# twogc/quic-test

Hardware: AMD Instinct MI355X
Metric: FEC encode+decode GiB/s (device-resident), k=10 r=3 1200B pkts, 1/2/4/8 GPU (higher is better)
Workload: dtype u8; 1 GPU; C2 encode + C3 decode: k=10 r=3, 1200 B packets, 1M groups/GPU, 2 erasures/group; k=10, r=3, packet_bytes=1200, groups_per_gpu=1000000, erasures_per_group=2, decode_api=fec_recover_batch_rs_dev (rebuilt packets at (g*r + m)*P slots), parallelism=group-sharded x1 (no collective)

## Files before the change

### quic-test_amd/csrc/fec_kernels.hip

```cpp
#include <hip/hip_runtime.h>

#include <cstdint>
#include <cstdlib>
#include <type_traits>

#include "bitslice.hpp"
#include "coef_tables.hpp"
#include "fec_kernels.hpp"
#include "fec_knobs.hpp"

namespace qfec {
namespace {

struct Tab {
  uint32_t t0lo, t0hi, t1lo, t1hi, t2, coef, p0, p1;
};

typedef uint32_t u32x4 __attribute__((ext_vector_type(4)));
typedef uint32_t u32x4u __attribute__((ext_vector_type(4), aligned(1)));
typedef uint32_t u32u __attribute__((aligned(1)));


template <int POL>
__device__ __forceinline__ u32x4 ld16(const uint8_t* p) {
// ... 462 lines not shown
      for (uint32_t b = 0; b < kBatch; ++b)
        if (s0 + b < k) consume(v[b], s0 + b, k);
    }
  }
#pragma unroll
  for (int m = 0; m < MAXE; ++m) {
    if (m0 + m < e) {
      const uint32_t eid = (POL & kCompactOut) != 0 ? m0 + m : rec_byte(rw, 64 + m0 + m);
      stw<NW, POL>(og + eid * static_cast<uint64_t>(P) + off, acc[m]);
    }
  }
}

template <int K, int MAXE, int POL, int NM, int NT, bool DIRECT, bool INLINE>
__device__ __forceinline__ void fused_group(uint64_t gw, uint64_t m, uint32_t lane, const uint8_t* __restrict__ data,
                                            const uint8_t* __restrict__ parity,
                                            const uint32_t* __restrict__ rec_off,
                                            const uint8_t* __restrict__ codebook, uint32_t P, uint32_t r,
                                            uint32_t m0, uint8_t* __restrict__ out, const RankMeta& rm,
                                            uint8_t* __restrict__ status) {
  constexpr int NW = 4 * NM + NT;
  constexpr uint64_t kmask = (1ull << K) - 1;
  uint64_t rec_byte_off;
  if constexpr (INLINE) {
    uint64_t dm = m & kmask;
    const uint64_t rmask = (1ull << r) - 1;
    const uint64_t pm = (m >> K) & rmask;
    const uint32_t ne = static_cast<uint32_t>(__popcll(dm));
    const bool bad = ne > r - static_cast<uint32_t>(__popcll(pm));
    if (status != nullptr && lane == 0) status[gw] = bad ? 1 : 0;
    if (ne == 0 || bad) return;
    uint64_t rank_e = 0, rank_r = 0;
    for (uint32_t t = 0; dm; ++t) {
      rank_e += choose_small(static_cast<uint32_t>(__builtin_ctzll(dm)), t + 1u);
      dm &= dm - 1;
    }
    uint64_t sp = ~pm & rmask;
    for (uint32_t t = 0; t < ne; ++t) {
      rank_r += choose_small(static_cast<uint32_t>(__builtin_ctzll(sp)), t + 1u);
      sp &= sp - 1;
    }
    rec_byte_off = rm.base[ne] + (rank_e * rm.count_r[ne] + rank_r) * rm.stride[ne];
  } else {
    const uint32_t rec = __builtin_amdgcn_readfirstlane(rec_off[gw]);
    if (rec >= kRecBad) return;
    rec_byte_off = static_cast<uint64_t>(rec) * 32u;
  }
  const uint8_t* recp = codebook + rec_byte_off;
  const uint32_t* rw = reinterpret_cast<const uint32_t*>(recp);
  uint32_t e;
  bool xor_only;
  uint64_t surv = 0, lost = 0;
  if constexpr (DIRECT) {
    lost = m & kmask;
    e = static_cast<uint32_t>(__popcll(lost));
    uint64_t alive = ~(m >> K) & ((r >= 64 ? 0ull : (1ull << r)) - 1);
    xor_only = e == 1 && (alive & 1u);
    uint64_t rsel = 0;
    for (uint32_t t = 0; t < e; ++t) {
      rsel |= alive & (~alive + 1);
      alive &= alive - 1;
    }
    surv = (~lost & kmask) | (rsel << K);
  } else {
    e = rw[24] & 0xFFu;
    xor_only = ((rw[24] >> 8) & 0xFFu) != 0;
  }
  if (m0 >= e) return;
  const Tab* tabs = reinterpret_cast<const Tab*>(recp + 128);
  const uint8_t* dg = data + gw * K * static_cast<uint64_t>(P);
  const uint8_t* pg = parity + gw * r * static_cast<uint64_t>(P);
  uint8_t* og = out + gw * K * static_cast<uint64_t>(P);
  const uint32_t main_end = NM * 1024u;
  uint32_t toff[NT > 0 ? NT : 1];
#pragma unroll
  for (int t = 0; t < NT; ++t) {
    toff[t] = main_end + t * 256u + lane * 4u;
    if (toff[t] + 4u > P) toff[t] = P - 4u;
  }
  auto load = [&](const uint8_t* base, uint32_t (&v)[NW]) {
#pragma unroll
    for (int i = 0; i < NM; ++i) {
      const u32x4 t = ld16<POL>(base + i * 1024u + lane * 16u);
      v[4 * i] = t.x;
      v[4 * i + 1] = t.y;
      v[4 * i + 2] = t.z;
      v[4 * i + 3] = t.w;
    }
#pragma unroll
    for (int t = 0; t < NT; ++t) {
      if constexpr ((POL & kNtLoad) != 0) v[4 * NM + t] = __builtin_nontemporal_load(reinterpret_cast<const u32u*>(base + toff[t]));
      else v[4 * NM + t] = *reinterpret_cast<const u32u*>(base + toff[t]);
    }
  };
  auto store = [&](uint8_t* base, const uint32_t (&v)[NW]) {
#pragma unroll
    for (int i = 0; i < NM; ++i) st16<POL>(base + i * 1024u + lane * 16u, u32x4{v[4 * i], v[4 * i + 1], v[4 * i + 2], v[4 * i + 3]});
#pragma unroll
    for (int t = 0; t < NT; ++t) {
      if constexpr ((POL & kNtStore) != 0) __builtin_nontemporal_store(v[4 * NM + t], reinterpret_cast<u32u*>(base + toff[t]));
      else *reinterpret_cast<u32u*>(base + toff[t]) = v[4 * NM + t];
    }
  };
  auto shard = [&](uint32_t sid) {
    return sid < K ? dg + sid * static_cast<uint64_t>(P) : pg + (sid - K) * static_cast<uint64_t>(P);
  };
  uint32_t sid[K];
#pragma unroll
  for (int s = 0; s < K; ++s) {
    if constexpr (DIRECT) {
      sid[s] = static_cast<uint32_t>(__builtin_ctzll(surv));
      surv &= surv - 1;
    } else {
      sid[s] = rec_byte(rw, s);
    }
  }
  auto dest = [&](uint32_t m, uint32_t eid) -> uint8_t* {
    if constexpr ((POL & kCompactOut) != 0) {
      uint64_t row = gw * r + m;
      if constexpr (INLINE) {
        if (rec_off != nullptr) row = static_cast<uint64_t>(__builtin_amdgcn_readfirstlane(rec_off[gw])) + m;
      }
      return out + row * static_cast<uint64_t>(P);
    } else {
      return og + eid * static_cast<uint64_t>(P);
    }
  };
  auto erased = [&](uint32_t m) -> uint32_t {
    if constexpr (DIRECT) {
      uint64_t x = lost;
      for (uint32_t t = 0; t < m; ++t) x &= x - 1;
      return static_cast<uint32_t>(__builtin_ctzll(x));
    } else {
      return rec_byte(rw, 64 + m);
    }
  };
  if (xor_only) {
    uint32_t acc[NW] = {};
#pragma unroll
    for (int s = 0; s < K; ++s) {
      uint32_t v[NW];
      load(shard(sid[s]), v);
#pragma unroll
      for (int q = 0; q < NW; ++q) acc[q] ^= v[q];
    }
    store(dest(0, erased(0)), acc);
    return;
  }
  constexpr bool kLds = (POL & kLdsTabs) != 0;
  constexpr int kTabPieces = MAXE * K * 2;
  constexpr int kTabIter = kLds ? (kTabPieces + 63) / 64 : 1;
  const uint32_t tab_pieces = (e - m0 < MAXE ? e - m0 : MAXE) * K * 2u;
  constexpr int kSliceTabs = kTabIter * 64 / 2;
  constexpr int kCoefIter = (MAXE * K + 63) / 64;
  uint32_t coef[kCoefIter];
  if constexpr (kLds && (POL & kCoefBytes) != 0) {
    const uint8_t* cb = recp + 128 + m0 * K;
    const uint32_t ncoef = tab_pieces / 2u;
#pragma unroll
    for (int j = 0; j < kCoefIter; ++j) {
      const uint32_t i = lane + 64u * j;
      coef[j] = i < ncoef ? cb[i] : 0u;
    }
  } else if constexpr (kLds) {
    const uint8_t* src = reinterpret_cast<const uint8_t*>(tabs + m0 * K);
    uint8_t* dst = reinterpret_cast<uint8_t*>(wave_tabs_lds<kSliceTabs>());
#pragma unroll
    for (int i = 0; i < kTabIter; ++i) {
      uint32_t idx = lane + 64u * i;
      if (idx >= tab_pieces) idx = tab_pieces - 1u;
      __builtin_amdgcn_global_load_lds(reinterpret_cast<const void*>(src + idx * 16u),
                                       (__attribute__((address_space(3))) void*)(dst + i * 1024), 16, 0, 0);
    }
  }
  constexpr bool kWinPath = kLds;
  constexpr int kWinW = 6;
  constexpr int kWin = kWinPath ? (K < kWinW ? K : kWinW) : K;
  uint32_t x[K][NW];
#pragma unroll
  for (int s = 0; s < kWin; ++s) load(shard(sid[s]), x[s]);
  if constexpr (kLds && (POL & kCoefBytes) != 0) {
    Tab* lt = wave_tabs_lds<kSliceTabs>();
    const uint32_t ncoef = tab_pieces / 2u;
#pragma unroll
    for (int j = 0; j < kCoefIter; ++j) {
      const uint32_t i = lane + 64u * j;
      if (i < ncoef) {
        const TabWords w = tab_words(coef[j]);
        lt[i] = Tab{w.t0lo, w.t0hi, w.t1lo, w.t1hi, w.t2, coef[j], 0u, 0u};
      }
    }
  }
  const Tab* rt = tabs + m0 * K;
  if constexpr (kWinPath) {
    const Tab* lt = rt;
    if constexpr (kLds) {
      __builtin_amdgcn_s_waitcnt(0x0F70);
      __builtin_amdgcn_fence(__ATOMIC_ACQUIRE, "wavefront");
      __builtin_amdgcn_wave_barrier();
      lt = wave_tabs_lds<kSliceTabs>();
    }
    auto rebuild = [&](auto nr_c) __attribute__((always_inline)) {
      constexpr int NR = decltype(nr_c)::value;
      uint32_t acc[NR][NW];
#pragma unroll
      for (int m = 0; m < NR; ++m)
#pragma unroll
        for (int q = 0; q < NW; ++q) acc[m][q] = 0;
#pragma unroll
      for (int s = 0; s < K; ++s) {
#pragma unroll
        for (int q = 0; q < NW; ++q) __asm__ volatile("" : "+v"(x[s][q]));
        __builtin_amdgcn_sched_barrier(0);
        if (s + kWin < K) load(shard(sid[s + kWin]), x[s + kWin]);
        uint32_t s0[NW], s1[NW], s2[NW];
#pragma unroll
        for (int q = 0; q < NW; ++q) {
          s0[q] = x[s][q] & 0x07070707u;
          s1[q] = (x[s][q] >> 3) & 0x07070707u;
          s2[q] = (x[s][q] >> 6) & 0x03030303u;
        }
#pragma unroll
        for (int m = 0; m < NR; ++m) {
          const Tab t = lt[m * K + s];
#pragma unroll
          for (int q = 0; q < NW; ++q) {
            acc[m][q] ^= gmul(s0[q], s1[q], s2[q], t);
            __asm__ volatile("" : "+v"(acc[m][q]));
          }
        }
      }
#pragma unroll
      for (int m = 0; m < NR; ++m) store(dest(m0 + m, erased(m0 + m)), acc[m]);
    };
    for_row_count<MAXE>(e - m0 < MAXE ? e - m0 : MAXE, rebuild);
    return;
  } else {
#pragma unroll
    for (int s = kWin; s < K; ++s) load(shard(sid[s]), x[s]);
  }
  uint32_t acc[MAXE][NW];
#pragma unroll
  for (int m = 0; m < MAXE; ++m)
#pragma unroll
    for (int q = 0; q < NW; ++q) acc[m][q] = 0;
#pragma unroll
  for (int s = 0; s < K; ++s) {
    uint32_t s0[NW], s1[NW], s2[NW];
#pragma unroll
    for (int q = 0; q < NW; ++q) {
      s0[q] = x[s][q] & 0x07070707u;
      s1[q] = (x[s][q] >> 3) & 0x07070707u;
      s2[q] = (x[s][q] >> 6) & 0x03030303u;
    }
#pragma unroll
    for (int m = 0; m < MAXE; ++m) {
      if (m0 + m < e) {
        const Tab& t = rt[m * K + s];
        if (t.coef == 1u) {
#pragma unroll
          for (int q = 0; q < NW; ++q) acc[m][q] ^= x[s][q];
        } else if (t.coef != 0u) {
#pragma unroll
          for (int q = 0; q < NW; ++q) acc[m][q] ^= gmul(s0[q], s1[q], s2[q], t);
        }
      }
    }
  }
#pragma unroll
  for (int m = 0; m < MAXE; ++m)
    if (m0 + m < e) store(dest(m0 + m, erased(m0 + m)), acc[m]);
}

template <int K, int MAXE, int POL, int NM, int NT, bool DIRECT = false, bool INLINE = DIRECT, int SCAN = 0>
__global__ __launch_bounds__(256) void decode_fused(const uint8_t* __restrict__ data,
                                                    const uint8_t* __restrict__ parity,
                                                    const uint32_t* __restrict__ rec_off,
                                                    const uint8_t* __restrict__ codebook,
                                                    uint64_t groups, uint32_t P, uint32_t r, uint32_t m0,
                                                    uint8_t* __restrict__ out, uint32_t never, uint32_t swz,
                                                    const uint64_t* __restrict__ masks, RankMeta rm,
                                                    uint8_t* __restrict__ status) {
  static_assert(!INLINE || (DIRECT && MAXE <= 3), "inline classify: mask-addressed forms with r <= 3");
  static_assert(SCAN == 0 || (DIRECT && INLINE && (SCAN <= 64 || SCAN % 256 == 0)),
                "scan: mask-addressed inline forms, <= 64 groups per wave or whole 256-group rows per block");
  extern __shared__ __attribute__((aligned(16))) uint8_t occupancy_lds[];
  if (never) occupancy_lds[threadIdx.x] = 0;
  const uint64_t wv = static_cast<uint64_t>(decode_block(swz)) * 4u +
                      static_cast<uint32_t>(__builtin_amdgcn_readfirstlane(threadIdx.x >> 6));
  const uint32_t lane = threadIdx.x & 63u;
  if constexpr (SCAN > 64) {
    constexpr int J = SCAN / 256;
    __shared__ uint64_t seg_mask[SCAN];
    __shared__ uint16_t seg_idx[SCAN];
    __shared__ uint32_t seg_cnt[J * 4];
    const uint64_t g0 = static_cast<uint64_t>(decode_block(swz)) * SCAN;
    if (g0 >= groups) return;
    const uint32_t wave = static_cast<uint32_t>(__builtin_amdgcn_readfirstlane(threadIdx.x >> 6));
    constexpr uint64_t kmask = (1ull << K) - 1;
    uint64_t mv[J], bal[J];
#pragma unroll
    for (int j = 0; j < J; ++j) {
      const uint64_t g = g0 + j * 256u + threadIdx.x;
      bool need = false;
      mv[j] = 0;
      if (g < groups) {
        mv[j] = masks[g];
        const uint32_t ne = static_cast<uint32_t>(__popcll(mv[j] & kmask));
        const bool bad = ne > r - static_cast<uint32_t>(__popcll((mv[j] >> K) & ((1ull << r) - 1)));
        if (status != nullptr) status[g] = bad ? 1 : 0;
        need = ne > 0 && !bad;
      }
      bal[j] = __ballot(need);
      if (lane == 0) seg_cnt[j * 4 + wave] = static_cast<uint32_t>(__popcll(bal[j]));
    }
    __syncthreads();
    uint32_t total = 0, off[J];
#pragma unroll
    for (int c = 0; c < J * 4; ++c) {
      if (static_cast<uint32_t>(c % 4) == wave) off[c / 4] = total;
      total += seg_cnt[c];
    }
    const uint64_t below = (1ull << lane) - 1;
#pragma unroll
    for (int j = 0; j < J; ++j) {
      if ((bal[j] >> lane) & 1u) {
        const uint32_t pos = off[j] + static_cast<uint32_t>(__popcll(bal[j] & below));
        seg_mask[pos] = mv[j];
        seg_idx[pos] = static_cast<uint16_t>(j * 256u + threadIdx.x);
      }
    }
    __syncthreads();
    for (uint32_t i = wave; i < total; i += 4u) {
      const uint64_t mi = seg_mask[i];
      const uint64_t m = (static_cast<uint64_t>(__builtin_amdgcn_readfirstlane(static_cast<uint32_t>(mi >> 32))) << 32) |
                         __builtin_amdgcn_readfirstlane(static_cast<uint32_t>(mi));
      const uint32_t gl = __builtin_amdgcn_readfirstlane(static_cast<uint32_t>(seg_idx[i]));
      fused_group<K, MAXE, POL, NM, NT, DIRECT, INLINE>(g0 + gl, m, lane, data, parity, rec_off, codebook, P, r, m0,
                                                        out, rm, nullptr);
    }
  } else if constexpr (SCAN == 0) {
    if (wv >= groups) return;
    const uint64_t m = DIRECT ? masks[wv] : 0;
    fused_group<K, MAXE, POL, NM, NT, DIRECT, INLINE>(wv, m, lane, data, parity, rec_off, codebook, P, r, m0, out, rm,
                                                      status);
  } else {
    const uint64_t g0 = wv * SCAN;
    if (g0 >= groups) return;
    uint64_t mv = 0;
    bool need = false;
    if (lane < static_cast<uint32_t>(SCAN) && g0 + lane < groups) {
      mv = masks[g0 + lane];
      constexpr uint64_t kmask = (1ull << K) - 1;
      const uint32_t ne = static_cast<uint32_t>(__popcll(mv & kmask));
      const bool bad = ne > r - static_cast<uint32_t>(__popcll((mv >> K) & ((1ull << r) - 1)));
      if (status != nullptr) status[g0 + lane] = bad ? 1 : 0;
      need = ne > 0 && !bad;
    }
    uint64_t work = __ballot(need);
    while (work) {
      const uint32_t b = static_cast<uint32_t>(__builtin_ctzll(work));
      work &= work - 1;
      const uint64_t m = (static_cast<uint64_t>(__builtin_amdgcn_readlane(static_cast<uint32_t>(mv >> 32), b)) << 32) |
                         __builtin_amdgcn_readlane(static_cast<uint32_t>(mv), b);
      fused_group<K, MAXE, POL, NM, NT, DIRECT, INLINE>(g0 + b, m, lane, data, parity, rec_off, codebook, P, r, m0,
                                                        out, rm, nullptr);
    }
  }

}

constexpr uint64_t kRunAgg = 1ull << 32;
constexpr uint64_t kRunIncl = 2ull << 32;
constexpr uint32_t kRunEpochShift = 34;

struct RunMeta {
  const Tab* tabs;
// ... 1072 lines not shown
  if (tile == 0) return hipErrorInvalidValue;
  const uint32_t bs = (tile * cpp + 63) / 64 * 64;
  return for_chunks(a.groups, max_wave_blocks() * 2 * tile, [&](uint64_t g0, uint64_t gn) {
    const uint32_t blocks = static_cast<uint32_t>((gn + 2 * tile - 1) / (2 * tile));
    constexpr int kDefWaves = (POL & kStageRows) != 0 ? 10 : 0;
    const int waves = a.waves_per_cu ? a.waves_per_cu : knob(TestKnob::kEncodeWaves, kDefWaves);
    uint32_t smem = occupancy_cap_lds(waves, bs / 64);
    if constexpr ((POL & kStageRows) != 0) smem = std::max<uint32_t>(smem, 2 * tile * R * a.P);
    LaunchRecord t = launch_record(LaunchForm::kEncodeBits, blocks, bs, g0, gn);
    t.k = K, t.r = R, t.off = 0, t.pol = POL, t.tile = tile, t.aux = W;
    trace_launch(t);
    hipLaunchKernelGGL((encode_bits<K, R, W, POL>), dim3(blocks), dim3(bs), smem, s, a.data, a.parity, g0, cpp, a.P,
                       tile, gn, 0u);
  });
}

template <int OFF>
hipError_t run_encode_generic(const EncodeLaunch& a, hipStream_t s) {
  if (a.P < kVecMinP) {
    return for_chunks(a.groups, groups_per_launch(a.P), [&](uint64_t g0, uint64_t gn) {
      const uint32_t n = static_cast<uint32_t>(gn * a.P);
      LaunchRecord t = launch_record(LaunchForm::kEncodeBytes, blocks_for(n), 256, g0, gn);
      t.k = 0, t.off = OFF;
      trace_launch(t);
      hipLaunchKernelGGL(encode_bytes<OFF>, dim3(blocks_for(n)), dim3(256), 0, s, a.data, a.offsets,
                         a.parity, g0, n, a.P, a.k, a.r, static_cast<const Tab*>(a.tables));
    });
  }
  for (uint32_t row0 = 0; row0 < a.r; row0 += 8) {
    const uint32_t rows = (a.r - row0 < 8) ? a.r - row0 : 8;
    hipError_t e = hipSuccess;
#define QFEC_PASS(RR)                                                            \
  case RR:                                                                       \
    e = row0 == 0 ? run_encode_v16<0, RR, OFF, true>(a, row0, s)                 \
                  : run_encode_v16<0, RR, OFF, false>(a, row0, s);               \
    break;
    switch (rows) {
      QFEC_PASS(1)
      QFEC_PASS(2)
      QFEC_PASS(3)
      QFEC_PASS(4)
      QFEC_PASS(5)
      QFEC_PASS(6)
      QFEC_PASS(7)
      QFEC_PASS(8)
      default:
        return hipErrorInvalidValue;
    }
#undef QFEC_PASS
    if (e != hipSuccess) return e;
  }
  return hipSuccess;
}

}

hipError_t launch_encode(const EncodeLaunch& a, hipStream_t s) {
  if (a.groups == 0) return hipSuccess;
  const EncodeForm f = encode_form(a);
  if (f.K == 0)
    return f.OFF == 0 ? run_encode_generic<0>(a, s) : f.OFF == 1 ? run_encode_generic<1>(a, s)
         : f.OFF == 2 ? run_encode_generic<2>(a, s) : run_encode_generic<3>(a, s);
#define QFEC_V16(KK, RR, OO, PP)                                                              \
  if (f.kernel == EncodeKernel::kV16 && f.K == KK && f.R == RR && f.OFF == OO && f.POL == (PP)) \
    return run_encode_v16<KK, RR, OO, true, PP>(a, 0, s);
#define QFEC_BITS(KK, RR, OO, PP)                                                              \
  if (f.kernel == EncodeKernel::kBits && f.K == KK && f.R == RR && f.OFF == OO && f.POL == (PP)) \
    return run_encode_bits<KK, RR, 4, PP>(a, s);
  QFEC_ENCODE_V16_FORMS(QFEC_V16)
  QFEC_ENCODE_BITS_FORMS(QFEC_BITS)
#undef QFEC_BITS
#undef QFEC_V16
  return hipErrorNotSupported;
}

namespace {

RankMeta rank_meta(const LevelMeta& m) {
  RankMeta rm{};
  for (int e = 1; e <= 3; ++e) rm.base[e] = m.base[e], rm.stride[e] = m.stride[e], rm.count_r[e] = m.count_r[e];
  return rm;
}

hipError_t run_classify(const DecodeLaunch& a, hipStream_t s) {
  return for_chunks(a.groups, max_launch_threads(), [&](uint64_t g0, uint64_t gn) {
    trace_launch(launch_record(LaunchForm::kClassify, blocks_for(gn), 256, g0, gn));
    hipLaunchKernelGGL(classify, dim3(blocks_for(gn)), dim3(256), 0, s, a.masks + g0, gn, a.k, a.r,
                       a.binom, a.meta, a.rec_off ? a.rec_off + g0 : nullptr, a.status ? a.status + g0 : nullptr);
  });
}

hipError_t run_decode_bytes(const DecodeLaunch& a, hipStream_t s) {
  return for_chunks(a.groups, groups_per_launch(a.P), [&](uint64_t g0, uint64_t gn) {
    const uint32_t n = static_cast<uint32_t>(gn * a.P);
    LaunchRecord t = launch_record(LaunchForm::kDecodeBytes, blocks_for(n), 256, g0, gn);
    t.k = 0, t.pol = a.compact_out ? kCompactOut : 0;
    trace_launch(t);
    hipLaunchKernelGGL(decode_bytes, dim3(blocks_for(n)), dim3(256), 0, s, a.data, a.parity,
                       a.rec_off, a.codebook, g0, n, a.P, a.k, a.r, a.out ? a.out : a.data,
                       a.compact_out ? 1u : 0u);
  });
}

template <int K, int MAXE>
hipError_t run_decode_v16(const DecodeLaunch& a, hipStream_t s) {
  const uint32_t cpp = (a.P + 15u) / 16u;
  const uint32_t passes = (a.r + MAXE - 1) / MAXE;
  for (uint32_t p = 0; p < passes; ++p) {
    const uint32_t m0 = p * MAXE;
    const hipError_t e = for_chunks(a.groups, max_wave_blocks() * 4, [&](uint64_t g0, uint64_t gn) {
      const uint64_t bn = (gn + 3) / 4;
      LaunchRecord t = launch_record(LaunchForm::kDecodeV16, bn, 256, g0, gn);
      t.k = K, t.r = MAXE, t.aux = m0;
      trace_launch(t);
      hipLaunchKernelGGL((decode_v16<K, MAXE>), dim3(static_cast<uint32_t>(bn)), dim3(256), 0, s,
                         a.data + g0 * a.k * static_cast<uint64_t>(a.P),
                         a.parity + g0 * a.r * static_cast<uint64_t>(a.P), a.rec_off ? a.rec_off + g0 : nullptr, a.codebook,
                         gn, cpp, a.P, a.k, a.r, m0);
    });
    if (e != hipSuccess) return e;
  }
  return hipSuccess;
}

template <int K, int MAXE, int POL>
hipError_t run_decode_wave(const DecodeLaunch& a, hipStream_t s) {
  const uint32_t passes = (a.r + MAXE - 1) / MAXE;
  const uint32_t cap = occupancy_cap_lds(a.waves_per_cu ? a.waves_per_cu : knob(TestKnob::kDecodeWaves, kDecodeWavesPerCU), 4);
  for (uint32_t p = 0; p < passes; ++p) {
    const uint32_t m0 = p * MAXE;
    const uint32_t rows = a.r - m0 < MAXE ? a.r - m0 : MAXE;
    const uint32_t slice = (POL & kLdsTabs) != 0 ? (rows * a.k * 2u + 63u) / 64u * 1024u : 0u;
    const uint32_t smem = cap > 4 * slice ? cap : 4 * slice;
    const hipError_t e = for_chunks(a.groups, max_wave_blocks() * 4, [&](uint64_t g0, uint64_t gn) {
      const uint64_t bn = (gn + 3) / 4;
      LaunchRecord t = launch_record(LaunchForm::kDecodeWave, bn, 256, g0, gn);
      t.k = K, t.r = MAXE, t.pol = POL, t.aux = m0;
      trace_launch(t);
      hipLaunchKernelGGL((decode_wave<K, MAXE, POL>), dim3(static_cast<uint32_t>(bn)), dim3(256), smem, s,
                         a.data + g0 * a.k * static_cast<uint64_t>(a.P),
                         a.parity + g0 * a.r * static_cast<uint64_t>(a.P), a.rec_off ? a.rec_off + g0 : nullptr, a.codebook, gn, a.P,
                         a.k, a.r, m0, (a.out ? a.out : a.data) + g0 * ((POL & kCompactOut) != 0 ? a.r : a.k) * static_cast<uint64_t>(a.P), 0u,
                         decode_swizzle(a, kDecodeWaveXcdSwizzle), slice);
    });
    if (e != hipSuccess) return e;
  }
  return hipSuccess;
}

template <int K, int MAXE, int POL, int NM, int NT, bool DIRECT = false, bool INLINE = DIRECT, int SCAN = 0>
hipError_t run_decode_fused(const DecodeLaunch& a, hipStream_t s) {
  constexpr uint64_t kGroupsPerBlock = SCAN > 64 ? SCAN : 4u * (SCAN > 0 ? SCAN : 1);
  const uint32_t passes = (a.r + MAXE - 1) / MAXE;
  const uint32_t smem = occupancy_cap_lds(a.waves_per_cu ? a.waves_per_cu : knob(TestKnob::kDecodeWaves, kDecodeWavesPerCU), 4);
  const RankMeta rm = rank_meta(a.meta);
  auto out_at = [&](uint64_t g0) -> uint8_t* {
    if (a.packed_rows) return a.out;
    return (a.out ? a.out : a.data) + g0 * ((POL & kCompactOut) != 0 ? a.r : a.k) * static_cast<uint64_t>(a.P);
  };
  for (uint32_t p = 0; p < passes; ++p) {
    const uint32_t m0 = p * MAXE;
    const hipError_t e = for_chunks(a.groups, max_wave_blocks() * kGroupsPerBlock, [&](uint64_t g0, uint64_t gn) {
      const uint64_t bn = (gn + kGroupsPerBlock - 1) / kGroupsPerBlock;
      LaunchRecord t = launch_record(LaunchForm::kDecodeFused, bn, 256, g0, gn);
      t.k = K, t.r = MAXE, t.nm = NM, t.nt = NT, t.pol = POL, t.direct = DIRECT, t.scan = SCAN, t.aux = m0;
      trace_launch(t);
      hipLaunchKernelGGL((decode_fused<K, MAXE, POL, NM, NT, DIRECT, INLINE, SCAN>), dim3(static_cast<uint32_t>(bn)), dim3(256), smem, s,
                         a.data + g0 * a.k * static_cast<uint64_t>(a.P),
                         a.parity + g0 * a.r * static_cast<uint64_t>(a.P), a.rec_off ? a.rec_off + g0 : nullptr, a.codebook, gn, a.P,
                         a.r, m0, out_at(g0), 0u, decode_swizzle(a, kDecodeFusedXcdSwizzle), DIRECT ? a.masks + g0 : nullptr, rm,
                         INLINE && a.status ? a.status + g0 : nullptr);
    });
    if (e != hipSuccess) return e;
  }
  return hipSuccess;
}

template <int K, int MAXE, int POL>
hipError_t run_decode_tiled(const DecodeLaunch& a, uint32_t tile, hipStream_t s) {
  const uint32_t cpp = (a.P + 15u) / 16u;
  const uint32_t bs = (tile * cpp + 63) / 64 * 64;
  return for_chunks(a.groups, groups_per_launch(bs) * tile, [&](uint64_t g0, uint64_t gn) {
    const uint64_t bn = (gn + tile - 1) / tile;
    LaunchRecord t = launch_record(LaunchForm::kDecodeTiled, bn, bs, g0, gn);
    t.k = K, t.r = MAXE, t.pol = POL, t.tile = tile;
    trace_launch(t);
    hipLaunchKernelGGL((decode_tiled<K, MAXE, POL>), dim3(static_cast<uint32_t>(bn)), dim3(bs), 0, s,
                       a.data + g0 * a.k * static_cast<uint64_t>(a.P),
                       a.parity + g0 * a.r * static_cast<uint64_t>(a.P), a.rec_off ? a.rec_off + g0 : nullptr, a.codebook, gn, cpp,
                       a.P, a.r, tile,
                       (a.out ? a.out : a.data) + g0 * ((POL & kCompactOut) != 0 ? a.r : a.k) * static_cast<uint64_t>(a.P));
  });
}

template <DecodeKernel KERNEL, int K, int MAXE, int NM, int NT, int POL, bool DIRECT, int SCAN>
hipError_t run_decode_form(const DecodeLaunch& a, uint32_t tile, hipStream_t s) {
  if constexpr (KERNEL == DecodeKernel::kFused) return run_decode_fused<K, MAXE, POL, NM, NT, DIRECT, DIRECT, SCAN>(a, s);
  else if constexpr (KERNEL == DecodeKernel::kTiled) return run_decode_tiled<K, MAXE, POL>(a, tile, s);
  else if constexpr (KERNEL == DecodeKernel::kWave) return run_decode_wave<K, MAXE, POL>(a, s);
  else if constexpr (KERNEL == DecodeKernel::kV16) return run_decode_v16<K, MAXE>(a, s);
  else return run_decode_bytes(a, s);
}

}

uint64_t rows_prefix_workspace_bytes(uint64_t groups) {
  return ((groups + kRowsPerBlock - 1) / kRowsPerBlock) * sizeof(uint32_t);
}

hipError_t launch_rows_prefix(const uint64_t* masks, uint64_t groups, uint32_t k, uint32_t r, uint32_t* row_start,
                              uint32_t* block_sums, uint64_t* total, hipStream_t s) {
  if (groups == 0) return hipSuccess;
  const uint64_t nb = (groups + kRowsPerBlock - 1) / kRowsPerBlock;
  if (nb > 0xFFFFFFFFull) return hipErrorInvalidValue;
  const uint64_t direct_max = static_cast<uint64_t>(knob(TestKnob::kRowsDirectBlocks, kRowsDirectBlocks));
  const dim3 grid(static_cast<uint32_t>(nb));
  const bool direct = nb <= direct_max;
  {
    trace_launch(launch_record(LaunchForm::kRowsBlockSums, nb, 256, 0, groups));
    if (!direct) trace_launch(launch_record(LaunchForm::kRowsScanBlocks, 1, 256, 0, groups));
    LaunchRecord t = launch_record(LaunchForm::kRowsWrite, nb, 256, 0, groups);
    t.direct = direct;
    trace_launch(t);
  }
  hipLaunchKernelGGL(rows_block_sums, grid, dim3(256), 0, s, masks, groups, k, r, block_sums);
  if (direct) {
    hipLaunchKernelGGL(rows_write<true>, grid, dim3(256), 0, s, masks, groups, k, r, block_sums, row_start, total);
  } else {
    hipLaunchKernelGGL(rows_scan_blocks, dim3(1), dim3(256), 0, s, block_sums, static_cast<uint32_t>(nb), total);
    hipLaunchKernelGGL(rows_write<false>, grid, dim3(256), 0, s, masks, groups, k, r, block_sums, row_start,
                       nullptr);
  }
  return hipGetLastError();
}

namespace {

constexpr int kRunWaves = 8;
constexpr uint32_t kRunGroups = 64u * kRunWaves;

uint64_t runs_blocks_per_launch(uint64_t groups) {
  const uint64_t nb = (groups + kRunGroups - 1) / kRunGroups;
  const uint64_t mb = max_wave_blocks();
  return nb < mb ? nb : mb;
}

template <int K, int R, int NM, int NT, int POL = kNtLoad | kNtStore>
hipError_t run_recover_runs(const RunsLaunch& a, uint32_t stage, hipStream_t s) {
  const RankMeta rm = rank_meta(a.meta);
  uint8_t* ws = static_cast<uint8_t*>(a.workspace);
  uint32_t* ticket = reinterpret_cast<uint32_t*>(ws);
  const uint64_t per = runs_blocks_per_launch(a.groups) * kRunGroups;
  const uint32_t launches = runs_launches(a.groups);
  uint64_t* totals = reinterpret_cast<uint64_t*>(ws + 64);
  uint64_t* lb = reinterpret_cast<uint64_t*>(ws + 64 + 8 * static_cast<uint64_t>(launches));
  return for_chunks(a.groups, per, [&](uint64_t g0, uint64_t gn) {
    const uint32_t c = static_cast<uint32_t>(g0 / per);
    const uint32_t nb = static_cast<uint32_t>((gn + kRunGroups - 1) / kRunGroups);
    LaunchRecord t = launch_record(LaunchForm::kRecoverRuns, nb, 64 * kRunWaves, g0, gn);
    t.k = K, t.r = R, t.nm = NM, t.nt = NT, t.pol = POL, t.tile = kRunGroups, t.aux = stage;
    trace_launch(t);
    hipLaunchKernelGGL((recover_runs<K, R, NM, NT, POL, kRunWaves>), dim3(nb), dim3(64 * kRunWaves), stage, s, a.data + g0 * K * static_cast<uint64_t>(a.P),
                       a.parity + g0 * R * static_cast<uint64_t>(a.P), a.masks + g0, gn, a.P, a.codebook, rm, a.out,
                       a.row_start + g0, a.status ? a.status + g0 : nullptr, lb, ticket, a.epoch + c, stage,
                       c > 0 ? totals + (c - 1) : nullptr, totals + c, c + 1 == launches ? a.total : nullptr, 0u);
  });
}

}

uint32_t runs_launches(uint64_t groups) {
  if (groups == 0) return 0;
  const uint64_t per = runs_blocks_per_launch(groups) * kRunGroups;
  return static_cast<uint32_t>((groups + per - 1) / per);
}

uint64_t runs_workspace_bytes(uint64_t groups) {
  return 64 + 8 * static_cast<uint64_t>(runs_launches(groups)) + 8 * runs_blocks_per_launch(groups);
}

uint32_t runs_stage_bytes(const RunsLaunch& a) {
  if (a.P % 16u != 0 || reinterpret_cast<uintptr_t>(a.out) % 16u != 0) return 0;
  const int v = a.stage_bytes >= 0 ? a.stage_bytes : knob(TestKnob::kRunsStage, kRunsStageBytes);
  if (v <= 0) return 0;
  const uint32_t cap = 64u * 1024u;
  return static_cast<uint32_t>(v) < cap ? static_cast<uint32_t>(v) : cap;
}

hipError_t launch_recover_runs(const RunsLaunch& a, hipStream_t s) {
  if (a.groups == 0) return hipSuccess;
  if (a.workspace == nullptr || a.row_start == nullptr || a.out == nullptr || a.masks == nullptr) return hipErrorInvalidValue;
  if (!runs_supported(a.k, a.r, a.P)) return hipErrorNotSupported;
  const Layout lay = layout_of(a.P);
#define QFEC_RUNS(KK, RR, NMM, NTT) \
  if (a.k == KK && a.r == RR && lay.nm == NMM && lay.nt == NTT) return run_recover_runs<KK, RR, NMM, NTT>(a, runs_stage_bytes(a), s);
  QFEC_RUNS_FORMS(QFEC_RUNS)
#undef QFEC_RUNS
  return hipErrorNotSupported;
}

hipError_t launch_decode(const DecodeLaunch& a, hipStream_t s) {
  const DecodeForm f = decode_form(a);
  if (f.kernel == DecodeKernel::kNone) return hipSuccess;
  if (a.compact_tables != f.compact_tables) return hipErrorInvalidValue;
  if (f.rec_off && a.rec_off == nullptr) return hipErrorInvalidValue;
  if (f.classify) {
    const hipError_t e = run_classify(a, s);
// ... 65 lines not shown
```

### quic-test_amd/csrc/fec_kernels.hpp

```cpp
#pragma once

#include <hip/hip_runtime.h>

#include <cstdint>

#include "fec_forms.hpp"

namespace qfec {

constexpr int kEncodeBlocksPerCU = 2;
constexpr int kEncodeXorWavesPerCU = 15;
constexpr int kDecodeWavesPerCU = 0;

inline uint32_t occupancy_cap_lds(int waves_per_cu, uint32_t waves_per_block) {
  if (waves_per_cu <= 0 || waves_per_block == 0) return 0;
  uint32_t blocks = (static_cast<uint32_t>(waves_per_cu) + waves_per_block / 2) / waves_per_block;
  if (blocks == 0) blocks = 1;
  if (blocks * waves_per_block >= 32) return 0;
  return 160u * 1024u / (blocks + 1) + 16u;
}

constexpr int kDecodeFusedXcdSwizzle = 1;
constexpr int kDecodeWaveXcdSwizzle = 1;

hipError_t launch_encode(const EncodeLaunch& a, hipStream_t s);
hipError_t launch_decode(const DecodeLaunch& a, hipStream_t s);
uint64_t rows_prefix_workspace_bytes(uint64_t groups);
hipError_t launch_rows_prefix(const uint64_t* masks, uint64_t groups, uint32_t k, uint32_t r, uint32_t* row_start,
                              uint32_t* block_sums, uint64_t* total, hipStream_t s);
constexpr int kRunsStageBytes = 48 * 1024;
uint32_t runs_launches(uint64_t groups);
uint64_t runs_workspace_bytes(uint64_t groups);
uint32_t runs_stage_bytes(const RunsLaunch& a);
hipError_t launch_recover_runs(const RunsLaunch& a, hipStream_t s);
constexpr uint32_t kServerSlots = 1024;
constexpr uint32_t kServerMaxGroups = 8;
constexpr uint32_t kServerPackets = 10;
constexpr uint64_t kServerTagShift = 48;
constexpr uint64_t kServerAddrMask = (1ull << kServerTagShift) - 1;
constexpr uint32_t kServerEpoch = 32768;
__host__ __device__ inline uint32_t server_tag(uint64_t seq, uint32_t epoch) {
  return (static_cast<uint32_t>(seq / kServerSlots) & (epoch - 1u)) + 1u;
}
__host__ __device__ inline bool server_scrub_after(uint64_t seq, uint32_t epoch) {
  return (static_cast<uint32_t>(seq / kServerSlots) & (epoch - 1u)) == epoch - 1u;
}
struct alignas(64) ServerSlot {
  uint64_t out;
  uint64_t shape;
  uint64_t addr[kServerMaxGroups * kServerPackets];
};
constexpr uint64_t kServerInline = 1ull << 24;
constexpr uint32_t kInlineMaxGroups = 4;
constexpr uint32_t kInlineMaxP = 1536;
constexpr uint32_t kInlinePayload = 12;
constexpr uint32_t kInlineSlotBytes = kInlineMaxGroups * kServerPackets * (kInlineMaxP / kInlinePayload) * 16;
constexpr uint32_t kServerMaxClasses = 8;
constexpr uint32_t kServerPoll = 16;
struct alignas(64) ServerControl {
  uint64_t stop;
  uint64_t pad0[7];
  uint64_t exited;
  uint64_t pad1[7];
  uint64_t progress[kServerMaxClasses];
  uint64_t bad_slots[kServerMaxClasses];
  uint64_t scrubs[kServerMaxClasses];
};
struct alignas(64) ServerCoord {
  uint64_t leave;
  uint64_t exits;
  uint64_t pad[6];
  uint64_t idle[kServerMaxClasses];
};
__host__ __device__ inline bool server_all_idle(bool idle, const uint64_t* idle_seen, uint32_t classes, uint32_t cls,
                                                uint64_t gen) {
  bool all = idle;
  for (uint32_t c = 0; c < classes; ++c) all = all && (c == cls || idle_seen[c] == gen);
  return all;
}
__host__ __device__ inline uint64_t server_exits_next(uint64_t v, uint64_t gen) {
  return (v >> 8) == gen ? v + 1 : (gen << 8) | 1u;
}
__host__ __device__ inline bool server_exits_last(uint64_t nv, uint32_t classes) { return (nv & 0xFFu) == classes; }
hipError_t launch_legacy_server(ServerSlot* ring, uint8_t* inl, uint64_t* done, ServerControl* ctl,
                                ServerCoord* coord, uint32_t classes, uint64_t gen, uint64_t idle_ticks,
                                uint64_t slow_ticks, uint64_t life_ticks, uint64_t* stamps, uint32_t epoch,
                                hipStream_t s);

hipError_t launch_fill_splitmix(uint8_t* dst, uint64_t nbytes, uint64_t seed, uint64_t byte_offset,
                                hipStream_t s);
hipError_t launch_copy_words(const uint8_t* src, uint8_t* dst, uint64_t nbytes, hipStream_t s);

constexpr uint32_t kRecNone = 0xFFFFFFFFu;
constexpr uint32_t kRecBad = 0xFFFFFFFEu;

}
```

Before: 2378 GiB/s.

## Hold decode GF tables in registers via readlane and cap fused-decode occupancy

For the non-LDS decode path with few table pieces, each lane loads one 16-byte table piece into a vector register. Per-source tables are then broadcast with readlane instead of being read from memory per row. The loop is restructured to compute the 3-bit slices per word once and apply them to all rebuilt rows. Separately, the fused decode for k=10, maxe=3 without LDS tables gets a tuned waves-per-CU cap of 12 via LDS padding, trading occupancy for more registers and cache per wave.

```diff
diff --git a/quic-test_amd/csrc/fec_kernels.hip b/quic-test_amd/csrc/fec_kernels.hip
--- a/quic-test_amd/csrc/fec_kernels.hip
+++ b/quic-test_amd/csrc/fec_kernels.hip
@@ -638,6 +638,12 @@
   constexpr int kTabIter = kLds ? (kTabPieces + 63) / 64 : 1;
   const uint32_t tab_pieces = (e - m0 < MAXE ? e - m0 : MAXE) * K * 2u;
   constexpr int kSliceTabs = kTabIter * 64 / 2;
+  constexpr bool kVecTabs = !kLds && kTabPieces <= 64;
+  u32x4 tv = {};
+  if constexpr (kVecTabs) {
+    const uint32_t idx = lane < tab_pieces ? lane : tab_pieces - 1u;
+    tv = *reinterpret_cast<const u32x4*>(reinterpret_cast<const uint8_t*>(tabs + m0 * K) + idx * 16u);
+  }
   constexpr int kCoefIter = (MAXE * K + 63) / 64;
   uint32_t coef[kCoefIter];
   if constexpr (kLds && (POL & kCoefBytes) != 0) {
@@ -659,9 +665,9 @@
                                        (__attribute__((address_space(3))) void*)(dst + i * 1024), 16, 0, 0);
     }
   }
-  constexpr bool kWinPath = kLds;
+  constexpr bool kWinPath = kLds || kVecTabs;
   constexpr int kWinW = 6;
-  constexpr int kWin = kWinPath ? (K < kWinW ? K : kWinW) : K;
+  constexpr int kWin = kLds ? (K < kWinW ? K : kWinW) : K;
   uint32_t x[K][NW];
 #pragma unroll
   for (int s = 0; s < kWin; ++s) load(shard(sid[s]), x[s]);
@@ -686,6 +692,14 @@
       __builtin_amdgcn_wave_barrier();
       lt = wave_tabs_lds<kSliceTabs>();
     }
+    auto tab_at = [&](int i) __attribute__((always_inline)) -> Tab {
+      if constexpr (kVecTabs) {
+        const auto word = [](uint32_t v, int l) { return static_cast<uint32_t>(__builtin_amdgcn_readlane(v, l)); };
+        return Tab{word(tv.x, 2 * i), word(tv.y, 2 * i), word(tv.z, 2 * i), word(tv.w, 2 * i), word(tv.x, 2 * i + 1), 0u, 0u, 0u};
+      } else {
+        return lt[i];
+      }
+    };
     auto rebuild = [&](auto nr_c) __attribute__((always_inline)) {
       constexpr int NR = decltype(nr_c)::value;
       uint32_t acc[NR][NW];
@@ -699,6 +713,22 @@
         for (int q = 0; q < NW; ++q) __asm__ volatile("" : "+v"(x[s][q]));
         __builtin_amdgcn_sched_barrier(0);
         if (s + kWin < K) load(shard(sid[s + kWin]), x[s + kWin]);
+        if constexpr (kVecTabs) {
+          Tab t[NR];
+#pragma unroll
+          for (int m = 0; m < NR; ++m) t[m] = tab_at(m * K + s);
+#pragma unroll
+          for (int q = 0; q < NW; ++q) {
+            const uint32_t a0 = x[s][q] & 0x07070707u, a1 = (x[s][q] >> 3) & 0x07070707u,
+                           a2 = (x[s][q] >> 6) & 0x03030303u;
+#pragma unroll
+            for (int m = 0; m < NR; ++m) {
+              acc[m][q] ^= gmul(a0, a1, a2, t[m]);
+              __asm__ volatile("" : "+v"(acc[m][q]));
+            }
+          }
+          continue;
+        }
         uint32_t s0[NW], s1[NW], s2[NW];
 #pragma unroll
         for (int q = 0; q < NW; ++q) {
@@ -708,7 +738,7 @@
         }
 #pragma unroll
         for (int m = 0; m < NR; ++m) {
-          const Tab t = lt[m * K + s];
+          const Tab t = tab_at(m * K + s);
 #pragma unroll
           for (int q = 0; q < NW; ++q) {
             acc[m][q] ^= gmul(s0[q], s1[q], s2[q], t);
@@ -2087,7 +2117,8 @@
 hipError_t run_decode_fused(const DecodeLaunch& a, hipStream_t s) {
   constexpr uint64_t kGroupsPerBlock = SCAN > 64 ? SCAN : 4u * (SCAN > 0 ? SCAN : 1);
   const uint32_t passes = (a.r + MAXE - 1) / MAXE;
-  const uint32_t smem = occupancy_cap_lds(a.waves_per_cu ? a.waves_per_cu : knob(TestKnob::kDecodeWaves, kDecodeWavesPerCU), 4);
+  constexpr int kTunedWaves = decode_fused_waves_per_cu(K, MAXE, POL, NM, SCAN);
+  const uint32_t smem = occupancy_cap_lds(a.waves_per_cu ? a.waves_per_cu : knob(TestKnob::kDecodeWaves, kTunedWaves), 4);
   const RankMeta rm = rank_meta(a.meta);
   auto out_at = [&](uint64_t g0) -> uint8_t* {
     if (a.packed_rows) return a.out;
diff --git a/quic-test_amd/csrc/fec_kernels.hpp b/quic-test_amd/csrc/fec_kernels.hpp
--- a/quic-test_amd/csrc/fec_kernels.hpp
+++ b/quic-test_amd/csrc/fec_kernels.hpp
@@ -11,6 +11,11 @@
 constexpr int kEncodeBlocksPerCU = 2;
 constexpr int kEncodeXorWavesPerCU = 15;
 constexpr int kDecodeWavesPerCU = 0;
+constexpr int kDecodeFusedWavesPerCU = 12;
+constexpr int decode_fused_waves_per_cu(int k, int maxe, int pol, int nm, int scan) {
+  return k == 10 && maxe == 3 && (pol & kLdsTabs) == 0 && nm >= 1 && scan == 0 ? kDecodeFusedWavesPerCU
+                                                                              : kDecodeWavesPerCU;
+}
 
 inline uint32_t occupancy_cap_lds(int waves_per_cu, uint32_t waves_per_block) {
   if (waves_per_cu <= 0 || waves_per_block == 0) return 0;
```

Result: slower. 2277 GiB/s (-4.2%).
